# fpthink/PDGN

Measured on AMD Instinct MI355X. Metric: generator+D step points/sec (B=35, 256->2048 pts), higher is better.
Workload: dtype f32; 1 GPU; PDGNet_v2 G+D iteration (models/PDGNet_v2.py:171-256), chair-shaped synthetic batch, per-GPU batch 35, 256->2048 pts, random-init weights; global_batch=35, parallelism=dp1, losses_finite=True, hipgraph=False, issue=list

## Files before the change

include/pdgn_hip.h:

```cpp
#ifndef PDGN_HIP_H
#define PDGN_HIP_H

#include <stdint.h>

#ifdef __cplusplus
extern "C" {
#endif

#define PDGN_ERR_INVALID (-1)
#define PDGN_KNN_MAX_NSAMPLE 200

typedef void *pdgn_stream_t;

#define PDGN_ABI_VERSION 38
int pdgn_abi_version(void);

int pdgn_knnquery(int b, int n, int m, int nsample, const float *xyz, const float *new_xyz,
                  int32_t *idx, float *dist2, pdgn_stream_t stream);

int pdgn_grouping_forward(int b, int c, int n, int m, int nsample, const float *points,
                          const int32_t *idx, float *out, pdgn_stream_t stream);

int pdgn_grouping_backward(int b, int c, int n, int m, int nsample, const float *grad_out,
                           const int32_t *idx, float *grad_points, pdgn_stream_t stream);
// ... 89 lines not shown
int pdgn_dense_bn_maxpool_input_grad(int b, int n, int c, int k, int act, const float *x, const float *dout,
                                     const int32_t *yarg, const float *stats, const float *h, int ldh,
                                     const float *W, int ldw, float *scratch, float *dh, pdgn_stream_t stream);

int pdgn_group_colsum(long long groups, long long group_rows, int c, const float *x, long long ldx, float *out,
                      pdgn_stream_t stream);

int pdgn_softmax_slots_permute(long long m, int k, int c, const float *h, float *w, pdgn_stream_t stream);
int pdgn_bn_softmax_slots_permute(long long m, int k, int c, int act, const float *x, const float *stats,
                                  float *w, pdgn_stream_t stream);
int pdgn_bn_softmax_slots_permute_mul(long long m, int k, int c, int act, const float *x, const float *stats,
                                      int act_u, const float *u, const float *stats_u, float *w, float *y,
                                      unsigned *max_out, const float *gamma_u, const float *beta_u, float bound_scale,
                                      unsigned *cmax_out, pdgn_stream_t stream);
long long pdgn_bilateral_scratch_floats(long long m, int k, int c);
int pdgn_bilateral_weighting_backward(long long m, int k, int c, int act, int training, const float *x,
                                      const float *stats_x, const float *u, const float *stats_u, const float *w,
                                      const float *dy, float *scratch, float *bsums_x, float *bsums_u, float *dx,
                                      float *du, pdgn_stream_t stream);
int pdgn_softmax_slots_permute_backward(long long m, int k, int c, const float *w, const float *dw,
                                        float *dh, pdgn_stream_t stream);

int pdgn_skinny_nt(int R, int N, int K, const float *A, int lda, const float *B, int ldb, const float *bias, float *C, int ldc,
                   pdgn_stream_t stream);
int pdgn_skinny_nn(int R, int N, int K, const float *A, int lda, const float *B, int ldb, float *C, int ldc, pdgn_stream_t stream);
int pdgn_skinny_nt_act(int R, int N, int K, const float *A, int lda, const float *B, int ldb, const float *bias, float *C, int ldc,
                       int act, pdgn_stream_t stream);
int pdgn_skinny_nn_masked(int R, int N, int K, const float *A, int lda, const float *P, int ldp, int act, const float *B,
                          int ldb, float *C, int ldc, pdgn_stream_t stream);
int pdgn_skinny_tn(int R, int N, int K, const float *A, int lda, const float *B, int ldb, float *C, int ldc, pdgn_stream_t stream);
int pdgn_split_bf16x3(int rows, int cols, const float *src, int ld_src, unsigned short *planes, int ld_planes,
                      long long plane_stride, unsigned short *planes_t, int ld_planes_t, long long plane_stride_t,
                      pdgn_stream_t stream);
int pdgn_gemm_nt_ps(long long m, int n, int k, const float *A, int lda, const unsigned short *Wplanes, int ldw, long long wplane,
                    int parts, const float *bias, const float *addend, int ldadd, float *C, int ldc, float *stat_part,
                    const float *row_bias, int ld_rb, int rows_per_group, int act, const float *gate, int ldgate,
                    pdgn_stream_t stream);
long long pdgn_gemm_tail_workspace_floats(long long m, int n, int k, int with_stats);
long long pdgn_gemm_tn_big_workspace_floats(long long m, int n, int k);
int pdgn_gemm_set_tail_workspace(float *ws, long long floats);
int pdgn_gemm_nt_ps_launch_info(long long m, int n, int k, int parts, const void **sym, int *grid);
int pdgn_gemm_aux_symbols(const void **reduce, const void **scan);
int pdgn_gemm_set_mode(int mode);
int pdgn_gemm_set_scale_slots(void *slots, long long bytes);
int pdgn_absmax_rows_cols(long long rows, int cols, const float *src, int ld, unsigned *rowmax, unsigned *colmax,
                          pdgn_stream_t stream);
int pdgn_gemm_set_operand_scales(const unsigned *max_a, const unsigned *max_w);
int pdgn_gemm_two_part(long long m, int n, int k, long long scan_bytes);
int pdgn_gemm_two_part_planes(long long m, int n, int k, long long scan_bytes);
long long pdgn_gemm_nt_ps_stat_rows(long long m, int n, int k, int parts, int plain);
int pdgn_gemm_nt_ps_stat_block_rows(long long m, int n, int k, int parts, int plain);
int pdgn_gemm_nt_ps_row_panel(long long m, int n, int k, int parts, int plain);
long long pdgn_gemm_nt_ps_workspace_floats(long long m, int n, int k, int parts, int with_stats);
int pdgn_split_f16x2(int rows, int cols, const float *src, int ld_src, unsigned short *planes, int ld_planes,
                     long long plane_stride, unsigned short *planes_t, int ld_planes_t, long long plane_stride_t,
                     pdgn_stream_t stream);
int pdgn_gemm_set_config(int cfg);
int pdgn_gemm_set_shape(int shape);
int pdgn_gemm_nt(long long m, int n, int k, const float *A, int lda, const float *W, int ldw,
                 const float *bias, const float *addend, int ldadd, float *C, int ldc, float *stat_part,
                 pdgn_stream_t stream);
long long pdgn_thin_stat_rows(long long m);
int pdgn_thin_stat_block_rows(void);
int pdgn_thin_nt(long long m, int n, int k, const float *X, int ldx, const float *W, int wrs, int wcs,
                 const float *bias, float *Y, int ldy, float *stat_part, pdgn_stream_t stream);
int pdgn_thin_nt_ex(long long m, int n, int k, const float *X, int ldx, const float *W, int wrs, int wcs,
                    const float *bias, float *Y, int ldy, float *stat_part, const float *gate, int ldgate, pdgn_stream_t stream);
int pdgn_thin_tn(long long m, int ta, int wb, const float *A, int lda, const float *B, int ldb, float *O, int osi,
                 int osj, float *sum_a, float *sum_b, pdgn_stream_t stream);
int pdgn_gemm_nn(long long m, int n, int k, const float *A, int lda, const float *Wt, int ldw,
                 const float *bias, const float *addend, int ldadd, float *C, int ldc, float *stat_part,
                 pdgn_stream_t stream);
int pdgn_gemm_tn_big(long long m, int n, int k, const float *dY, int ldy, const float *X, int ldx, float *dW, int dw_is_zero,
                     pdgn_stream_t stream);
int pdgn_gemm_nt_ex(long long m, int n, int k, const float *A, int lda, const float *W, int ldw, const float *bias,
                    const float *addend, int ldadd, float *C, int ldc, float *stat_part, const float *row_bias, int ld_rb,
                    int rows_per_group, int act, const float *gate, int ldgate, int transposed_w, pdgn_stream_t stream);
long long pdgn_gemm_nt_stat_rows(long long m, int n, int k);
int pdgn_gemm_nt_stat_block_rows(long long m, int n, int k);
int pdgn_gemm_nt_config(long long m, int n, int k, int with_stats);

int pdgn_gemm_tn(long long m, int n, int k, const float *dY, const float *X, float *dW,
                 pdgn_stream_t stream);

int pdgn_local_stats(int b, int n, int m, int k, const float *xyz, const int32_t *idx, float *mu,
                     float *cov, pdgn_stream_t stream);
int pdgn_local_stats_backward(int b, int n, int m, int k, const float *xyz, const int32_t *idx,
                              const float *dmu, const float *dcov, float *dxyz, pdgn_stream_t stream);

int pdgn_chamfer_gram(int b, int m, int n, int d, const float *x, const float *y, float *minx,
                      int32_t *argx, float *miny, int32_t *argy, pdgn_stream_t stream);
int pdgn_chamfer_gram_grad(int b, int m, int n, int d, const float *x, const float *y,
                           const float *gminx, const int32_t *argx, const float *gminy,
                           const int32_t *argy, float *gx, float *gy, pdgn_stream_t stream);
int pdgn_chamfer_gram_grad_uniform(int b, int m, int n, int d, const float *x, const float *y, const float *g,
                                   float scale, const int32_t *argx, const int32_t *argy, float *gx, float *gy,
                                   pdgn_stream_t stream);
int pdgn_scaled_sum(long long n, const float *x, float scale, float *out, pdgn_stream_t stream);
int pdgn_mse_const(long long n, const float *x, float target, float scale, float *out, pdgn_stream_t stream);
int pdgn_mse_const_count(long long n, const float *x, float target, float scale, float boundary, float *out, int32_t *count,
                         pdgn_stream_t stream);
int pdgn_mse_const_backward(long long n, const float *x, float target, float scale, const float *g, float *dx,
                            pdgn_stream_t stream);

int pdgn_emd_cost_indexed(int npairs, int n, int m, const float *xyz1, const int32_t *ia,
                          const float *xyz2, const int32_t *ib, float *temp, float *out,
                          pdgn_stream_t stream);
int pdgn_chamfer_gram_indexed(int npairs, int m, int n, int d, const float *x, const int32_t *ia,
                              const float *y, const int32_t *ib, float *minx, int32_t *argx,
                              float *miny, int32_t *argy, pdgn_stream_t stream);

int pdgn_deconv_assemble(int F, int Fo, int k, int T, int fc, const float *Wi, const float *W2, const float *Wf,
                         float *WcatC, float *WcatV, float *Wb, pdgn_stream_t stream);
int pdgn_deconv_assemble_backward(int F, int Fo, int k, int T, int fc, const float *gWcatC, const float *gWcatV,
                                  const float *gWb, float *dWi, float *dW2, float *dWf, pdgn_stream_t stream);

int pdgn_sample_bias(int b, int ldy, int nspec, const int *T, const int *C, const int *off, const int *offc,
                     const float *const *bias, const float *Yc, float *bb, pdgn_stream_t stream);
int pdgn_sample_bias_backward(int b, int ldy, int nspec, const int *T, const int *C, const int *off, const int *offc,
                              const float *g, float *dYc, float *const *dbias, pdgn_stream_t stream);

int pdgn_small_mlp_forward(int r, int k, int n, int act, int bn_mode, float eps, float momentum, const float *x,
                           const float *W, const float *bias, const float *gamma, const float *beta,
                           float *running_mean, float *running_var, float *y, float *pre, float *stat,
                           pdgn_stream_t stream);
int pdgn_small_mlp_backward(int r, int k, int n, int act, int bn_mode, const float *x, const float *dy, const float *pre,
                            const float *stat, const float *gamma, const float *beta, float *dpre, float *dgamma,
                            float *dbeta, float *dbias, float *dW, pdgn_stream_t stream);

int pdgn_ballquery(int b, int n, int m, float radius, int nsample, const float *new_xyz, const float *xyz,
                   int32_t *idx, pdgn_stream_t stream);
int pdgn_furthestsampling(int b, int n, int m, const float *xyz, float *temp, int32_t *idx, pdgn_stream_t stream);
int pdgn_gathering_forward(int b, int c, int n, int m, const float *points, const int32_t *idx, float *out,
                           pdgn_stream_t stream);
int pdgn_gathering_backward(int b, int c, int n, int m, const float *grad_out, const int32_t *idx,
                            float *grad_points, pdgn_stream_t stream);
int pdgn_grouping_int_forward(int b, int c, int n, int m, int nsample, const long long *points, const int32_t *idx,
                              long long *out, pdgn_stream_t stream);
int pdgn_featuredistribute(int b, int n, int m, const float *max_xyz, const float *xyz, int32_t *distribute_idx,
                           pdgn_stream_t stream);
int pdgn_labelstat_idx(int b, int n, int m, int nsample, int nclass, const int32_t *label_stat, const int32_t *idx,
                       int32_t *new_label_stat, pdgn_stream_t stream);
int pdgn_labelstat_ballrange(int b, int n, int m, float radius, int nclass, const float *new_xyz, const float *xyz,
                             const int32_t *label_stat, int32_t *new_label_stat, pdgn_stream_t stream);
int pdgn_labelstat_and_ballquery(int b, int n, int m, float radius, int nsample, int nclass, const float *new_xyz,
                                 const float *xyz, const int32_t *label_stat, int32_t *idx, int32_t *new_label_stat,
                                 pdgn_stream_t stream);

long long pdgn_point_max_scratch(int b, int n, int c);
int pdgn_point_max(int b, int n, int c, const float *x, float *scratch_val, int32_t *scratch_arg, float *out, int32_t *arg,
                   pdgn_stream_t stream);
int pdgn_point_max_backward(int b, int n, int c, const float *grad_out, const int32_t *arg, float *grad_x,
                            pdgn_stream_t stream);

int pdgn_spin(unsigned int microseconds, pdgn_stream_t stream);

int pdgn_replay_marker(int id, pdgn_stream_t stream);
int pdgn_replay_build(void *hip_graph, void **plan_out);
int pdgn_replay_info(void *plan, int *counts8);
int pdgn_replay_chains(void *plan, int *labels, int *nodes_per_chain);
int pdgn_replay_set_stream(void *plan, int chain, pdgn_stream_t stream);
int pdgn_replay_launch(void *plan);
int pdgn_replay_launch_range(void *plan, int lo, int hi);
int pdgn_replay_position(void *plan, int chain, int nth);
int pdgn_replay_points(void *plan, int *ids, int *pos, int *chain, int max_out);
int pdgn_replay_joined(void *plan);
// ... 137 lines not shown
```

pdgn_amd/csrc/gemm_shared.h:

```cpp
#pragma once
#include <type_traits>

#include "common.h"

typedef float f32x4 __attribute__((ext_vector_type(4)));
typedef unsigned u32x4 __attribute__((ext_vector_type(4)));
typedef __attribute__((address_space(3))) void lds_void_t;

#define NT_BK 32
#define NT_GROUP_M 8
#define NT_OOB 0x40000000u

typedef int i32x4 __attribute__((ext_vector_type(4)));

__device__ __forceinline__ i32x4 nt_srd(const void *base, unsigned bytes) {
    const unsigned long long b = (unsigned long long)base;
    i32x4 r;
    r.x = __builtin_amdgcn_readfirstlane((int)(unsigned)b);
    r.y = __builtin_amdgcn_readfirstlane((int)((unsigned)(b >> 32) & 0xffffu));
    r.z = __builtin_amdgcn_readfirstlane((int)bytes);
    r.w = 0x00020000;
    return r;
}

__device__ __forceinline__ void nt_dma16(i32x4 srd, unsigned lds_base, unsigned voff, unsigned soff) {
    asm volatile("s_mov_b32 m0, %0\n\ts_nop 0\n\tbuffer_load_dwordx4 %1, %2, %3 offen lds"
                 :
                 : "s"(lds_base), "v"(voff), "s"(srd), "s"(soff)
                 : "memory", "m0");
}

struct NtArgs {
    long long M;
    int N, K, lda, ldw, ldc, ldadd;
    const float *A, *W, *bias, *addend;
    float *C, *stat_part;
    int tiles_m, tiles_n, tile_begin, tile_end, kchunks;
    long long sk_per_wg;
    int sk_split;
    float *sk_ws;
    int sk_seg;
    int dbg;
    const float *row_bias;
    int ld_rb, rows_per_group;
    unsigned rpg_magic;
    int rb_bytes;
    int act;
    const float *gate;
    int ldgate;
    const unsigned short *Wp;
    long long wplane;
    const unsigned *max_a, *max_w;
};

__device__ __forceinline__ int x2_exponent(unsigned maxbits) {
    const int e = 14 - ((int)(maxbits >> 23) - 127);
    return e > 126 ? 126 : (e < -126 ? -126 : e);
}
__device__ __forceinline__ int x2_scale_field(unsigned maxbits) {
    const int f = 268 - (int)(maxbits >> 23);
    return f < 1 ? 1 : (f > 253 ? 253 : f);
}
__device__ __forceinline__ float x2_scale(unsigned maxbits) { return __int_as_float(x2_scale_field(maxbits) << 23); }
__device__ __forceinline__ float x2_unscale(unsigned maxbits) { return __int_as_float((254 - x2_scale_field(maxbits)) << 23); }

struct NtDev {
    int cus;
};
static inline int nt_cus() {
    static int cached = 0;
    if (!cached) {
        int dev = 0, cus = 0;
        if (hipGetDevice(&dev) != hipSuccess ||
            hipDeviceGetAttribute(&cus, hipDeviceAttributeMultiprocessorCount, dev) != hipSuccess || cus < 1)
            return 256;
        cached = cus;
    }
    return cached;
}

struct NtSwitches {
    int mode, cfg, splitk, shape16, shape16_default;
};
NtSwitches &nt_switches();

struct NtEpi {
    const float *row_bias = nullptr;
    int ld_rb = 0, rows_per_group = 1, act = 0;
    const float *gate = nullptr;
    int ldgate = 0;
    bool any() const { return row_bias || act || gate; }
};


int fp32_gemm_nt(long long m, int n, int k, const float *A, int lda, const float *W, int ldw, const float *bias,
                 const float *addend, int ldadd, float *C, int ldc, float *stat_part, pdgn_stream_t stream);
int fp32_gemm_nn(long long m, int n, int k, const float *A, int lda, const float *Wt, int ldw, const float *bias,
                 const float *addend, int ldadd, float *C, int ldc, float *stat_part, pdgn_stream_t stream);
int fp32_gemm_nt_ex(long long m, int n, int k, const float *A, int lda, const float *W, int ldw, const float *bias,
                    const float *addend, int ldadd, float *C, int ldc, float *stat_part, const float *row_bias, int ld_rb,
                    int rows_per_group, int act, const float *gate, int ldgate, int transposed_w, pdgn_stream_t stream);
int fp32_gemm_tn_big(long long m, int n, int k, const float *dY, int ldy, const float *X, int ldx, float *dW,
                     pdgn_stream_t stream);
long long fp32_gemm_nt_stat_rows(long long m, int n, int k);
int fp32_gemm_nt_stat_block_rows(long long m, int n, int k);
int fp32_gemm_nt_config(long long m, int n, int k, int with_stats);
```

pdgn_amd/csrc/gemm_x3.hip:

```cpp
#include <atomic>
#include <type_traits>

#include "gemm_shared.h"

#ifndef X3_FENCE
#define X3_FENCE 2
#endif
#ifndef X3_DEFAULT_MASK
#define X3_DEFAULT_MASK 0x000
#endif
#ifndef X3_FENCE16
#define X3_FENCE16 2
#endif
#ifndef X3_ABLATE
#define X3_ABLATE 0
#endif

typedef float f32x16 __attribute__((ext_vector_type(16)));
typedef float f32x2 __attribute__((ext_vector_type(2)));
typedef __bf16 bf16x8 __attribute__((ext_vector_type(8)));
typedef __bf16 bf16x2 __attribute__((ext_vector_type(2)));

struct X3Parts {
    u32x4 h, m, l;
};

__device__ __forceinline__ unsigned x3_cvt_pk(float a, float b) {
    const f32x2 v = {a, b};
    return __builtin_bit_cast(unsigned, __builtin_convertvector(v, bf16x2));
}

__device__ __forceinline__ void x3_split_pair(float a, float b, X3Parts &P, int e) {
    const unsigned h = x3_cvt_pk(a, b);
    const float ra = a - __uint_as_float(h << 16), rb = b - __uint_as_float(h & 0xffff0000u);
    const unsigned m = x3_cvt_pk(ra, rb);
    const float sa = ra - __uint_as_float(m << 16), sb = rb - __uint_as_float(m & 0xffff0000u);
    P.h[e] = h;
    P.m[e] = m;
    P.l[e] = x3_cvt_pk(sa, sb);
}

__device__ __forceinline__ f32x16 x3_mfma(const u32x4 a, const u32x4 b, const f32x16 c) {
    return __builtin_amdgcn_mfma_f32_32x32x16_bf16(__builtin_bit_cast(bf16x8, a), __builtin_bit_cast(bf16x8, b), c, 0, 0, 0);
}

typedef _Float16 f16x8 __attribute__((ext_vector_type(8)));
typedef _Float16 f16x2 __attribute__((ext_vector_type(2)));
__device__ __forceinline__ unsigned x2_cvt_pk(float a, float b) {
    const f32x2 v = {a, b};
    return __builtin_bit_cast(unsigned, __builtin_convertvector(v, f16x2));
}
__device__ __forceinline__ f32x16 x2_mfma(const u32x4 a, const u32x4 b, const f32x16 c) {
    return __builtin_amdgcn_mfma_f32_32x32x16_f16(__builtin_bit_cast(f16x8, a), __builtin_bit_cast(f16x8, b), c, 0, 0, 0);
}
#ifndef X2_PRODUCTS
#define X2_PRODUCTS 3
#endif

typedef float f32x4a __attribute__((ext_vector_type(4)));
__device__ __forceinline__ f32x4a x3_mfma16(const u32x4 a, const u32x4 b, const f32x4a c) {
    return __builtin_amdgcn_mfma_f32_16x16x32_bf16(__builtin_bit_cast(bf16x8, a), __builtin_bit_cast(bf16x8, b), c, 0, 0, 0);
}

template <int MS>
__device__ __forceinline__ unsigned x3_sw(unsigned r) {
    const unsigned x = (r >> 2) & 3u;
    return MS == 32 ? x : ((0x78u >> (2u * x)) & 3u);
}

template <int CTRL, int ROW_MASK>
__device__ __forceinline__ float x3_dpp_add(float v) {
    return v + __int_as_float(__builtin_amdgcn_update_dpp(0, __float_as_int(v), CTRL, ROW_MASK, 0xf, true));
}

__device__ __forceinline__ float x3_half_wave_sum(float v) {
    v = x3_dpp_add<0x111, 0xf>(v);
    v = x3_dpp_add<0x112, 0xf>(v);
    v = x3_dpp_add<0x114, 0xf>(v);
    v = x3_dpp_add<0x118, 0xf>(v);
    return x3_dpp_add<0x142, 0xa>(v);
}

__device__ __forceinline__ float x3_row_sum(float v) {
    v = x3_dpp_add<0x111, 0xf>(v);
    v = x3_dpp_add<0x112, 0xf>(v);
    v = x3_dpp_add<0x114, 0xf>(v);
    return x3_dpp_add<0x118, 0xf>(v);
}

template <int TM, int TN, int WM, int WN, int OCC, bool ATOMIC, bool WT, bool AT, bool EPI = false, bool PW = false, int MS = 32, int NP = 3>
__global__ __launch_bounds__(64 * WM * WN, OCC) void gemm_x3_kernel(const NtArgs p) {
    static_assert(!PW || (!WT && !AT), "pre-split second operand: row-major (N x K) planes only");
    static_assert(MS == 32 || MS == 16, "matrix instruction: 32x32x16 or 16x16x32");
    static_assert(NP == 3 || (NP == 2 && MS == 32), "parts: three bf16, or two fp16 on the 32x32x16 instruction");
    constexpr int NW = WM * WN, NTH = 64 * NW, BM = 32 * TM * WM, BN = 32 * TN * WN;
    constexpr int PART_A = BM * 64, PART_W = BN * 64, STAGE = NP * (PART_A + PART_W);
    constexpr int UNT = NP == 2 ? (BM + BN) * 4 : 0;
    constexpr bool STG = OCC == 1 && !ATOMIC && !(X3_ABLATE & 128) && 2 * STAGE + NW * 4096 + UNT <= 160 * 1024;
    __shared__ __attribute__((aligned(1024))) unsigned char smem[2 * STAGE + (STG ? NW * 4096 : 0) + UNT];
    float *const untab = reinterpret_cast<float *>(smem + 2 * STAGE + (STG ? NW * 4096 : 0));

    const int tid = threadIdx.x, lane = tid & 63;
    const int wave = __builtin_amdgcn_readfirstlane(tid >> 6);
    const int wm = wave / WN, wn = wave % WN;
    const int li = MS == 32 ? lane & 31 : lane & 15, lg = MS == 32 ? lane >> 5 : lane >> 4;

    const int G = gridDim.x, pid = blockIdx.x;
    const int gq = G >> 3, gr = G & 7, xcd = pid & 7;
    const int v = xcd * gq + min(xcd, gr) + (pid >> 3);

    const int KC = p.kchunks;
    auto decode = [&](int tile, int &tm, int &tn) {
        const int per_group = NT_GROUP_M * p.tiles_n;
        const int grp = tile / per_group, r = tile - grp * per_group;
        const int first = grp * NT_GROUP_M;
        const int gsz = min(NT_GROUP_M, p.tiles_m - first);
        tn = r / gsz;
        tm = first + (r - tn * gsz);
    };
    struct Cur {
        int tile, kb, kc, ke;
        int j;
        long long f, f1;
        bool valid;
    };
    auto next_item = [&](Cur &c) {
        if (p.sk_split && (ATOMIC || p.sk_ws)) {
// ... 1479 lines not shown
```

pdgn_amd/fused.py:

```python
import os
import weakref

import torch
from ._fn import Function

from . import _lib
from ._lib import check, ptr, require, stream_of

F32 = torch.float32
ACT = {"none": 0, "relu": 1, "leaky_relu": 2}


def _scratch_floats(L, rows, C):
    n = L.pdgn_bn_scratch_floats(rows, C)
    if n < 0:
        raise _lib.PdgnHipError("pdgn_bn_scratch_floats: argument outside the supported range")
    return n


_ZERO_COLSUM = {}


def mark_zero_colsum(dx):
    _ZERO_COLSUM[dx.data_ptr()] = weakref.ref(dx)
# ... 157 lines not shown
def _pre_bias_grad(ctx_has, C, device):
    return _zeros((C,), device) if ctx_has else None


class BNActCL(Function):

    @staticmethod
    def forward(ctx, x, gamma, beta, running_mean, running_var, training, momentum, eps, act, mul, pre_bias=None,
                partials=None, interleave_n=0):
        rows, C = x.shape
        x = x.contiguous()
        L = _lib.lib()
        g, b = gamma.detach().contiguous(), beta.detach().contiguous()
        stats = _bn_stats(L, x, rows, C, g, b, pre_bias, running_mean, running_var, training, momentum, eps, partials)
        ctx.has_pre_bias = pre_bias is not None
        mul_c = mul.contiguous() if mul is not None else None
        y = torch.empty((rows * 2, C // 2), dtype=F32, device=x.device) if interleave_n else torch.empty_like(x)
        check(L.pdgn_bn_act_forward(rows, C, act, ptr(x), ptr(stats), ptr(mul_c), ptr(y), int(interleave_n), stream_of(x)), "pdgn_bn_act_forward")
        ctx.save_for_backward(x, stats, mul_c)
        ctx.cfg = (rows, C, act, bool(training), mul is not None and mul.requires_grad, int(interleave_n))
        return y

    @staticmethod
    def backward(ctx, dy):
        x, stats, mul = ctx.saved_tensors
        rows, C, act, training, need_dmul, inter = ctx.cfg
        dy = dy.contiguous()
        L = _lib.lib()
        scratch = torch.empty(_scratch_floats(L, rows, C), dtype=F32, device=x.device)
        bs = torch.empty(2 * C, dtype=F32, device=x.device)
        dx = torch.empty_like(x)
        dmul = torch.empty_like(x) if need_dmul else None
        check(L.pdgn_bn_act_backward(rows, C, act, int(training), ptr(x), ptr(dy), ptr(mul),
                                     ptr(stats), ptr(scratch), ptr(bs), ptr(dx), ptr(dmul), inter, stream_of(x)), "pdgn_bn_act_backward")
        if training:
            mark_zero_colsum(dx)
        return (dx, bs[C:], bs[:C], None, None, None, None, None, None, dmul, _pre_bias_grad(ctx.has_pre_bias, C, x.device),
                None, None)


_PENDING_COUNTS = {}
_HOLD_COUNTS = [False]


def hold_bn_counters(on):
    old, _HOLD_COUNTS[0] = _HOLD_COUNTS[0], bool(on)
    return old


def flush_bn_counters():
    if _HOLD_COUNTS[0]:
        return
    if _PENDING_COUNTS:
        tensors = list(_PENDING_COUNTS.keys())
        torch._foreach_add_(tensors, [int(v) for v in _PENDING_COUNTS.values()])
        _PENDING_COUNTS.clear()


def bn_act(x2d, bn, training, act="leaky_relu", mul=None, pre_bias=None, partials=None, interleave_n=0):
    if training and bn.track_running_stats:
        _PENDING_COUNTS[bn.num_batches_tracked] = _PENDING_COUNTS.get(bn.num_batches_tracked, 0) + 1
    x2d, pre_bias = _fold_pre_bias(x2d, pre_bias, training)
    if x2d.shape[1] % 4:
        if pre_bias is not None:
            x2d = x2d + pre_bias
        y = torch.nn.functional.batch_norm(x2d, bn.running_mean, bn.running_var, bn.weight, bn.bias, training,
                                           bn.momentum, bn.eps)
        y = {"none": lambda t: t, "relu": torch.relu, "leaky_relu": torch.nn.functional.leaky_relu}[act](y)
        y = y * mul if mul is not None else y
        return interleave_rows(y, interleave_n) if interleave_n else y
    if interleave_n and (mul is not None or not x2d.is_cuda):
        return interleave_rows(bn_act(x2d, bn, training, act, mul, pre_bias, partials), interleave_n)
    return BNActCL.apply(x2d, bn.weight, bn.bias, bn.running_mean, bn.running_var, training, bn.momentum, bn.eps,
                         ACT[act], mul, pre_bias, partials, interleave_n)


def interleave_rows(y2d, n):
    rows, c2 = y2d.shape
    return y2d.view(rows // n, n, c2 // 2, 2).permute(0, 3, 1, 2).reshape(rows * 2, c2 // 2)


_OWN_MIN_ROWS = 1024
_TN_BIG = os.environ.get("PDGN_TN_BIG", "1") == "1"


def _tn_big_max():
    return (1 << 22) if _lib.matrix_core_mode() else (1 << 20)


def _pad_cols(t, mult=4):
    c = t.shape[1]
    if c % mult == 0 and t.stride(1) == 1 and t.stride(0) % 4 == 0 and t.data_ptr() % 16 == 0:
        return t
    if c % mult == 0:
        return t.contiguous()
    return torch.nn.functional.pad(t, (0, mult - c % mult)).contiguous()


GEMM_LOG = None


_PLANES = os.environ.get("PDGN_PLANES", "1") == "1"


class Planes:
    __slots__ = ("p", "t", "shape", "parts_p", "parts_t")

    def __init__(self, p, t, shape, parts_p=3, parts_t=3):
        self.p, self.t, self.shape, self.parts_p, self.parts_t = p, t, shape, parts_p, parts_t


def two_part(m, n, k, scan_bytes):
    return _lib.gemm_mode() == "x2" and bool(_lib.lib().pdgn_gemm_two_part(m, n, k, scan_bytes))


def two_part_planes(m, n, k, scan_bytes):
    return _lib.gemm_mode() == "x2" and bool(_lib.lib().pdgn_gemm_two_part_planes(m, n, k, scan_bytes))


def _slots(t):
    if _lib.gemm_mode() == "x2":
        _lib.ensure_scale_slots(t.device)


def split_planes(w, want_t, rows=None, dy_maxima_free=False, x_maxima_free=False):
    _slots(w)
    mode = _lib.gemm_mode()
    if (not (_PLANES and w.is_cuda and w.dim() == 2 and mode != "fp32") or w.shape[0] % 4 or w.shape[1] % 4 or w.stride(1) != 1
            or w.stride(0) % 4 or w.data_ptr() % 16):
        return None
    n, k = w.shape
    ldp, ldt = (k + 7) // 8 * 8, (n + 7) // 8 * 8
    parts_p = 2 if rows and two_part_planes(rows, n, k, 0 if x_maxima_free else rows * k * 4) else 3
    parts_t = 2 if rows and want_t and two_part_planes(rows, k, n, 0 if dy_maxima_free else rows * n * 4) else 3

    def planes(parts, rows_, ld):
        buf = torch.empty(parts * rows_ * ld + 2 * rows_ + 8, dtype=torch.int16, device=w.device)
        return buf[:parts * rows_ * ld].view(parts, rows_, ld)
    P = planes(parts_p, n, ldp)
    PT = planes(parts_t, k, ldt) if want_t else None
    L = _lib.lib()
    st = stream_of(w)
    if parts_p == parts_t or not want_t:
        fn = L.pdgn_split_bf16x3 if parts_p == 3 else L.pdgn_split_f16x2
        check(fn(n, k, ptr(w), w.stride(0), ptr(P), ldp, n * ldp, ptr(PT), ldt, k * ldt if want_t else 0, st), "pdgn_split")
    else:
        for parts, args in ((parts_p, (ptr(P), ldp, n * ldp, None, 0, 0)),
                            (parts_t, (None, 0, 0, ptr(PT), ldt, k * ldt))):
            fn = L.pdgn_split_bf16x3 if parts == 3 else L.pdgn_split_f16x2
            check(fn(n, k, ptr(w), w.stride(0), *args, st), "pdgn_split")
    return Planes(P, PT, (n, k), parts_p, parts_t)


def _maxima_ok(t):
    return (_lib.gemm_mode() == "x2" and t.is_cuda and t.dim() == 2 and t.stride(1) == 1 and t.dtype == F32 and t.shape[1] % 4 == 0
            and t.stride(0) % 4 == 0 and t.data_ptr() % 16 == 0)


def operand_maxima(t, rows=True, cols=False):
    if not _maxima_ok(t) or not (rows or cols):
        return (None, None) if (rows and cols) else None
    rm = torch.empty((t.shape[0],), dtype=torch.int32, device=t.device) if rows else None
    cm = torch.empty((t.shape[1],), dtype=torch.int32, device=t.device) if cols else None
    check(_lib.lib().pdgn_absmax_rows_cols(t.shape[0], t.shape[1], ptr(t), t.stride(0), ptr(rm), ptr(cm), stream_of(t)), "pdgn_absmax_rows_cols")
    return (rm, cm) if (rows and cols) else (rm if rows else cm)

# ... 9 lines not shown

def _tail_workspace(L, m, n, k, with_stats, device, parts=None):
    if parts is not None:
        need = L.pdgn_gemm_nt_ps_workspace_floats(m, n, k, parts, 1 if with_stats else 0)
    else:
        need = L.pdgn_gemm_tail_workspace_floats(m, n, k, 1 if with_stats else 0)
    if need <= 0:
        return None
    ws = torch.empty(need, dtype=F32, device=device)
    check(L.pdgn_gemm_set_tail_workspace(ptr(ws), need), "pdgn_gemm_set_tail_workspace")
    return ws


def _rp_takes(m, n, k, parts, plain):
    return parts == 2 and plain and _lib.lib().pdgn_gemm_nt_ps_row_panel(m, n, k, 2, 1) == 1


def planes_fit(P, m, n, k, with_stats=False, plain=False):
    return (P.shape[0] == 3 or not with_stats or _rp_takes(m, n, k, P.shape[0], plain) or (_lib.lib().pdgn_gemm_nt_config(m, n, k, 1) & 15) == 0)


def gemm_nt_planes(a, P, n, k, bias=None, addend=None, want_stats=False, max_a=None):
    _slots(a)
    m = a.shape[0]
    if GEMM_LOG is not None:
        GEMM_LOG.append(("nt", m, n, k))
    ap = _pad_cols(a)
    L = _lib.lib()
    out = torch.empty((m, n), dtype=F32, device=a.device)
    part = None
    if want_stats:
        part = torch.empty((L.pdgn_gemm_nt_ps_stat_rows(m, n, k, P.shape[0], 1 if (bias is None and addend is None) else 0),
                            3 * n), dtype=F32, device=a.device)
    b = bias.detach().contiguous() if bias is not None else None
    if addend is not None:
        addend = _pad_cols(addend)
    ws = _tail_workspace(L, m, n, k, want_stats, a.device, parts=P.shape[0])
    _hand_maxima(L, max_a)
    check(L.pdgn_gemm_nt_ps(m, n, k, ptr(ap), ap.stride(0), ptr(P), P.shape[2], P.shape[1] * P.shape[2], P.shape[0],
                            ptr(b), ptr(addend), addend.stride(0) if addend is not None else 0, ptr(out), n, ptr(part), None, 0, 1, 0,
                            None, 0, stream_of(a)), "pdgn_gemm_nt_ps")
    return (out, part) if want_stats else out


def gemm_nt(a, w, bias=None, addend=None, want_stats=False, w_transposed=False, max_a=None):
    _slots(a)
    m, k = a.shape
    n = w.shape[1] if w_transposed else w.shape[0]
    if GEMM_LOG is not None:
        GEMM_LOG.append(("nn" if w_transposed else "nt", m, n, k))
    ap = _pad_cols(a)
    kp = ap.shape[1]
    np_ = (n + 3) // 4 * 4
    if w_transposed:
        wp = _pad_cols(w)
        if kp != k:
            wp = torch.nn.functional.pad(wp, (0, 0, 0, kp - k))
    else:
        wp = _pad_cols(w)
    if np_ != n and not w_transposed:
        wp = torch.nn.functional.pad(wp, (0, 0, 0, np_ - n))
    if np_ != n:
        bias = torch.nn.functional.pad(bias, (0, np_ - n)) if bias is not None else None
        addend = torch.nn.functional.pad(addend, (0, np_ - n)) if addend is not None else None
    if addend is not None:
        addend = _pad_cols(addend)
    L = _lib.lib()
    out = torch.empty((m, np_), dtype=F32, device=a.device)
    part = None
    if want_stats:
        part = torch.empty((L.pdgn_gemm_nt_stat_rows(m, np_, kp), 3 * np_), dtype=F32, device=a.device)
    b = bias.detach().contiguous() if bias is not None else None
    fn = L.pdgn_gemm_nn if w_transposed else L.pdgn_gemm_nt
    ws = _tail_workspace(L, m, np_, kp, want_stats, a.device)
    _hand_maxima(L, max_a)
    check(fn(m, np_, kp, ptr(ap), ap.stride(0), ptr(wp), wp.stride(0), ptr(b), ptr(addend),
             addend.stride(0) if addend is not None else 0, ptr(out), np_, ptr(part), stream_of(a)),
          "pdgn_gemm_nn" if w_transposed else "pdgn_gemm_nt")
    if np_ != n:
        out = out[:, :n].contiguous()
    return (out, part) if want_stats else out


def gemm_tn(dy, x, max_dy=None, max_x=None):
    _slots(dy)
    m, n = dy.shape
    k = x.shape[1]
    if GEMM_LOG is not None:
        GEMM_LOG.append(("tn", m, n, k))
    dyp, xp = _pad_cols(dy), _pad_cols(x)
    nk = dyp.shape[1] * xp.shape[1]
    if _TN_BIG and dyp.shape[1] >= 64 and xp.shape[1] >= 64 and (65536 if (m < 150000 or not _lib.matrix_core_mode()) else 16384) <= nk <= _tn_big_max():
        L = _lib.lib()
        need = L.pdgn_gemm_tn_big_workspace_floats(m, dyp.shape[1], xp.shape[1])
        if need > 0:
            ws = torch.empty(need, dtype=F32, device=dy.device)
            check(L.pdgn_gemm_set_tail_workspace(ptr(ws), need), "pdgn_gemm_set_tail_workspace")
            dwp = torch.empty((dyp.shape[1], xp.shape[1]), dtype=F32, device=dy.device)
        else:
            dwp = _zeros((dyp.shape[1], xp.shape[1]), dy.device)
        _hand_maxima(L, max_dy, max_x)
        check(_lib.lib().pdgn_gemm_tn_big(m, dyp.shape[1], xp.shape[1], ptr(dyp), dyp.stride(0), ptr(xp),
                                          xp.stride(0), ptr(dwp), 0 if need > 0 else 1, stream_of(dy)), "pdgn_gemm_tn_big")
        return dwp if (dyp.shape[1] == n and xp.shape[1] == k) else dwp[:n, :k]
    if dyp.stride(0) != dyp.shape[1]:
        dyp = dyp.contiguous()
    if xp.stride(0) != xp.shape[1]:
        xp = xp.contiguous()
    dwp = _zeros((dyp.shape[1], xp.shape[1]), dy.device)
    check(_lib.lib().pdgn_gemm_tn(m, dyp.shape[1], xp.shape[1], ptr(dyp), ptr(xp), ptr(dwp), stream_of(dy)), "pdgn_gemm_tn")
    return dwp if (dyp.shape[1] == n and xp.shape[1] == k) else dwp[:n, :k]


def _thin_ok(x, n, k):
    return (k <= 4 and n % 4 == 0 and n <= 1024) or (n <= 4 and k % 4 == 0 and k <= 1024)


def thin_nt(x, w, wrs, wcs, n, bias=None, want_stats=False):
    m, k = x.shape
    if GEMM_LOG is not None:
        GEMM_LOG.append(("thin", m, n, k))
    x = x if (x.stride(1) == 1 and (k <= 4 or (x.stride(0) % 4 == 0 and x.data_ptr() % 16 == 0))) else x.contiguous()
    L = _lib.lib()
    out = torch.empty((m, n), dtype=F32, device=x.device)
    part = None
    if want_stats and k <= 4:
        part = torch.empty((L.pdgn_thin_stat_rows(m), 3 * n), dtype=F32, device=x.device)
    b = bias.detach().contiguous() if bias is not None else None
    check(L.pdgn_thin_nt(m, n, k, ptr(x), x.stride(0), ptr(w), wrs, wcs, ptr(b), ptr(out), n, ptr(part), stream_of(x)), "pdgn_thin_nt")
    return (out, part) if want_stats else out


def thin_tn(dy, x, want_db):
    m, n = dy.shape
    k = x.shape[1]
    if GEMM_LOG is not None:
        GEMM_LOG.append(("thin_tn", m, n, k))
    dw = _zeros((n, k), dy.device)
    db = _zeros((n,), dy.device) if want_db else None
    L = _lib.lib()
    if k <= 4:
        check(L.pdgn_thin_tn(m, k, n, ptr(x), x.stride(0), ptr(dy), dy.stride(0), ptr(dw), 1, k, ptr(None), ptr(db), stream_of(dy)), "pdgn_thin_tn")
    else:
        check(L.pdgn_thin_tn(m, n, k, ptr(dy), dy.stride(0), ptr(x), x.stride(0), ptr(dw), k, 1, ptr(db), ptr(None), stream_of(dy)), "pdgn_thin_tn")
    return dw, db


def _planes_taken(x, weight, planes, want_stats, plain):
    return (planes is not None and x.is_cuda and x.shape[0] >= _PLANES_MIN_ROWS and planes.shape == tuple(weight.shape)
            and x.shape[1] == weight.shape[1] and x.shape[1] % 4 == 0
            and planes_fit(planes.p, x.shape[0], weight.shape[0], weight.shape[1], want_stats, plain))


class LinearCL(Function):

    @staticmethod
    def forward(ctx, x, weight, bias, addend, want_stats=False, planes=None, x_max=None, x_cmax=None):
        ctx.save_for_backward(x, weight)
        ctx.set_materialize_grads(False)
        ctx.has_bias = bias is not None
        ctx.has_addend = addend is not None
        ctx.planes_t = None
        ctx.max_x = None
        ctx.max_x_cols = x_cmax
        if _planes_taken(x, weight, planes, want_stats, bias is None and addend is None):
            n, k = weight.shape
            ctx.thin = False
            ctx.planes_t = planes.t
            xm = None
            if planes.parts_p == 2 and not _rp_takes(x.shape[0], n, k, 2, bias is None and addend is None):
                xm = x_max if x_max is not None else operand_maxima(x)
            ctx.max_x = xm
            if want_stats:
                y, part = gemm_nt_planes(x, planes.p, n, k, bias, addend, want_stats=True, max_a=xm)
                ctx.mark_non_differentiable(part)
                return y, part
            return gemm_nt_planes(x, planes.p, n, k, bias, addend, max_a=xm)
        ctx.thin = bool(x.is_cuda and x.shape[0] >= _OWN_MIN_ROWS and addend is None and weight.is_contiguous()
                        and _thin_ok(x, weight.shape[0], weight.shape[1]))
        if ctx.thin:
            n, k = weight.shape
            if want_stats and k <= 4:
                y, part = thin_nt(x, weight, k, 1, n, bias, want_stats=True)
                ctx.mark_non_differentiable(part)
                return y, part
            y = thin_nt(x, weight, k, 1, n, bias)
# ... 646 lines not shown
```

Measured before the change: 3.147 million points/s.

## Add split-K bf16x3 MFMA weight-gradient GEMM for small TN shapes

Adds a new TN GEMM kernel for weight gradients outside the existing big-TN route. It splits each fp32 input into three bf16 parts and accumulates six MFMA cross products, which aims for near-fp32 accuracy on the matrix cores. It also splits the long M reduction across workgroups, writing to a workspace that a separate reduce kernel sums. The goal is to replace the old scalar pdgn_gemm_tn path with better CU occupancy and matrix-core throughput, at the cost of an extra reduction launch, workspace allocation and conversion work.

After: 3.145 million points/s. Within noise of the previous version (-0.1%).

```diff
diff --git a/include/pdgn_hip.h b/include/pdgn_hip.h
--- a/include/pdgn_hip.h
+++ b/include/pdgn_hip.h
@@ -195,6 +195,10 @@
 
 int pdgn_gemm_tn(long long m, int n, int k, const float *dY, const float *X, float *dW,
                  pdgn_stream_t stream);
+int pdgn_gemm_tn_sp(long long m, int n, int k, const float *dY, int ldy, const float *X, int ldx, float *dW, int lddw,
+                    float *workspace, long long workspace_floats, pdgn_stream_t stream);
+long long pdgn_gemm_tn_sp_workspace_floats(long long m, int n, int k);
+int pdgn_gemm_tn_sp_plan(long long m, int n, int k, int *tile_n, int *tile_k, int *splits, long long *rows_per_split);
 
 int pdgn_local_stats(int b, int n, int m, int k, const float *xyz, const int32_t *idx, float *mu,
                      float *cov, pdgn_stream_t stream);
diff --git a/pdgn_amd/csrc/gemm_shared.h b/pdgn_amd/csrc/gemm_shared.h
--- a/pdgn_amd/csrc/gemm_shared.h
+++ b/pdgn_amd/csrc/gemm_shared.h
@@ -64,6 +64,34 @@
 __device__ __forceinline__ float x2_scale(unsigned maxbits) { return __int_as_float(x2_scale_field(maxbits) << 23); }
 __device__ __forceinline__ float x2_unscale(unsigned maxbits) { return __int_as_float((254 - x2_scale_field(maxbits)) << 23); }
 
+typedef float f32x16 __attribute__((ext_vector_type(16)));
+typedef float f32x2 __attribute__((ext_vector_type(2)));
+typedef __bf16 bf16x8 __attribute__((ext_vector_type(8)));
+typedef __bf16 bf16x2 __attribute__((ext_vector_type(2)));
+
+struct X3Parts {
+    u32x4 h, m, l;
+};
+
+__device__ __forceinline__ unsigned x3_cvt_pk(float a, float b) {
+    const f32x2 v = {a, b};
+    return __builtin_bit_cast(unsigned, __builtin_convertvector(v, bf16x2));
+}
+
+__device__ __forceinline__ void x3_split_pair(float a, float b, X3Parts &P, int e) {
+    const unsigned h = x3_cvt_pk(a, b);
+    const float ra = a - __uint_as_float(h << 16), rb = b - __uint_as_float(h & 0xffff0000u);
+    const unsigned m = x3_cvt_pk(ra, rb);
+    const float sa = ra - __uint_as_float(m << 16), sb = rb - __uint_as_float(m & 0xffff0000u);
+    P.h[e] = h;
+    P.m[e] = m;
+    P.l[e] = x3_cvt_pk(sa, sb);
+}
+
+__device__ __forceinline__ f32x16 x3_mfma(const u32x4 a, const u32x4 b, const f32x16 c) {
+    return __builtin_amdgcn_mfma_f32_32x32x16_bf16(__builtin_bit_cast(bf16x8, a), __builtin_bit_cast(bf16x8, b), c, 0, 0, 0);
+}
+
 struct NtDev {
     int cus;
 };
diff --git a/pdgn_amd/csrc/gemm_tn_sp.hip b/pdgn_amd/csrc/gemm_tn_sp.hip
--- /dev/null
+++ b/pdgn_amd/csrc/gemm_tn_sp.hip
@@ -0,0 +1,324 @@
+#include "gemm_shared.h"
+
+typedef short sp_s16x4 __attribute__((ext_vector_type(4)));
+typedef __attribute__((address_space(3))) sp_s16x4 sp_lds_s16x4;
+
+#define SP_THREADS 256
+#define SP_MIN_ROWS 64
+#define SP_MAX_BLOCKS 16
+
+struct SpArgs {
+    long long M, rows;
+    int N, K, ldy, ldx, lddw;
+    int tiles_n, tiles_k, splits;
+    int ws_ld;
+    long long ws_split;
+    const float *dY, *X;
+    float *dW, *ws;
+};
+
+__host__ __device__ constexpr int sp_pitch(int t) { return ((2 * t) % 256 == 64 || (2 * t) % 256 == 192) ? 2 * t : 2 * t + 64; }
+
+__device__ __forceinline__ void sp_split4(const float4 v, uint2 &h, uint2 &m, uint2 &l) {
+    X3Parts P;
+    x3_split_pair(v.x, v.y, P, 0);
+    x3_split_pair(v.z, v.w, P, 1);
+    h = make_uint2(P.h[0], P.h[1]);
+    m = make_uint2(P.m[0], P.m[1]);
+    l = make_uint2(P.l[0], P.l[1]);
+}
+
+template <int PITCH>
+__device__ __forceinline__ u32x4 sp_frag(const unsigned char *p) {
+    const sp_s16x4 lo = __builtin_amdgcn_ds_read_tr16_b64_v4i16((sp_lds_s16x4 *)p);
+    const sp_s16x4 hi = __builtin_amdgcn_ds_read_tr16_b64_v4i16((sp_lds_s16x4 *)(p + 4 * PITCH));
+    const uint2 a = __builtin_bit_cast(uint2, lo), b = __builtin_bit_cast(uint2, hi);
+    u32x4 r = {a.x, a.y, b.x, b.y};
+    return r;
+}
+
+template <int TN, int TK, int CH>
+__global__ __launch_bounds__(SP_THREADS, (TN / 32) * ((TK < 32 ? 32 : TK) / 32) >= SP_MAX_BLOCKS ? 3 : 4) void gemm_tn_sp_kernel(const SpArgs a) {
+    constexpr int TKB = TK < 32 ? 32 : TK;
+    constexpr int BN = TN / 32, BK = TKB / 32;
+    constexpr int WGN = (BN >= 4 && BK >= 4) ? 2 : (BN >= 4 ? 4 : (BK >= 8 ? 1 : BN));
+    constexpr int WGK = (4 / WGN) < BK ? (4 / WGN) : BK;
+    constexpr int WBN = BN / WGN, WBK = BK / WGK;
+    constexpr int PY = sp_pitch(TN), PX = sp_pitch(TKB);
+    constexpr int QY = TN / 4, QX = TK / 4;
+    constexpr int YSTEP = SP_THREADS / QY, XSTEP = SP_THREADS / QX;
+    constexpr int NY = (CH + YSTEP - 1) / YSTEP, NX = (CH + XSTEP - 1) / XSTEP;
+    static_assert(BN * BK <= SP_MAX_BLOCKS && WBN * WGN == BN && WBK * WGK == BK, "tile");
+    __shared__ __attribute__((aligned(16))) unsigned char Ys[3 * CH * PY];
+    __shared__ __attribute__((aligned(16))) unsigned char Xs[3 * CH * PX];
+
+    const int total = gridDim.x, pid = blockIdx.x;
+    const int q8 = total >> 3, r8 = total & 7, xcd = pid & 7, slot = pid >> 3;
+    const int v = xcd * q8 + min(xcd, r8) + slot;
+    const int tiles = a.tiles_n * a.tiles_k;
+    const int tile = v % tiles, split = v / tiles;
+    const int n0 = (tile % a.tiles_n) * TN, k0 = (tile / a.tiles_n) * TK;
+    const long long m_begin = (long long)split * a.rows;
+    const long long m_end = min(a.M, m_begin + a.rows);
+
+    const int tid = threadIdx.x, lane = tid & 63, wave = tid >> 6;
+    const int wn = wave / WGK, wk = wave % WGK;
+    const bool multiplies = wave < WGN * WGK;
+
+    const int yr = tid / QY, yq = tid % QY, xr = tid / QX, xq = tid % QX;
+    const bool ycol = n0 + 4 * yq < a.N, xcol = k0 + 4 * xq < a.K;
+    const float *pY = a.dY + (m_begin + yr) * a.ldy + n0 + 4 * yq;
+    const float *pX = a.X + (m_begin + xr) * a.ldx + k0 + 4 * xq;
+    float4 ry[NY], rx[NX];
+    auto prefetch = [&](long long m0, bool tail) {
+#pragma unroll
+        for (int i = 0; i < NY; ++i) {
+            const int row = yr + i * YSTEP;
+            const bool ok = row < CH && ycol && (!tail || m0 + row < m_end);
+            ry[i] = ok ? *reinterpret_cast<const float4 *>(pY + (long long)(i * YSTEP) * a.ldy) : make_float4(0.f, 0.f, 0.f, 0.f);
+        }
+#pragma unroll
+        for (int i = 0; i < NX; ++i) {
+            const int row = xr + i * XSTEP;
+            const bool ok = row < CH && xcol && (!tail || m0 + row < m_end);
+            rx[i] = ok ? *reinterpret_cast<const float4 *>(pX + (long long)(i * XSTEP) * a.ldx) : make_float4(0.f, 0.f, 0.f, 0.f);
+        }
+    };
+
+    f32x16 acc[WBN][WBK];
+#pragma unroll
+    for (int i = 0; i < WBN; ++i)
+#pragma unroll
+        for (int j = 0; j < WBK; ++j)
+#pragma unroll
+            for (int r = 0; r < 16; ++r) acc[i][j][r] = 0.f;
+
+    const int fg = lane >> 5, fc = (lane >> 4) & 1, fq = (lane >> 2) & 3, fp = lane & 3;
+    const unsigned char *fY = Ys + (8 * fg + fq) * PY + (32 * wn * WBN + 16 * fc + 4 * fp) * 2;
+    const unsigned char *fX = Xs + (8 * fg + fq) * PX + (32 * wk * WBK + 16 * fc + 4 * fp) * 2;
+
+    const long long span = m_end - m_begin;
+    const int nfull = (int)(span / CH), nchunk = (int)((span + CH - 1) / CH);
+    prefetch(m_begin, nfull == 0);
+    for (int c = 0; c < nchunk; ++c) {
+        __syncthreads();
+#pragma unroll
+        for (int i = 0; i < NY; ++i) {
+            const int row = yr + i * YSTEP;
+            if (row < CH) {
+                uint2 h, m, l;
+                sp_split4(ry[i], h, m, l);
+                unsigned char *d = Ys + row * PY + yq * 8;
+                *reinterpret_cast<uint2 *>(d) = h;
+                *reinterpret_cast<uint2 *>(d + CH * PY) = m;
+                *reinterpret_cast<uint2 *>(d + 2 * CH * PY) = l;
+            }
+        }
+#pragma unroll
+        for (int i = 0; i < NX; ++i) {
+            const int row = xr + i * XSTEP;
+            if (row < CH) {
+                uint2 h, m, l;
+                sp_split4(rx[i], h, m, l);
+                unsigned char *d = Xs + row * PX + xq * 8;
+                *reinterpret_cast<uint2 *>(d) = h;
+                *reinterpret_cast<uint2 *>(d + CH * PX) = m;
+                *reinterpret_cast<uint2 *>(d + 2 * CH * PX) = l;
+            }
+        }
+        __syncthreads();
+        pY += (long long)CH * a.ldy;
+        pX += (long long)CH * a.ldx;
+        if (c + 1 < nchunk) prefetch(m_begin + (long long)(c + 1) * CH, c + 1 >= nfull);
+        if (multiplies) {
+#pragma unroll
+            for (int s = 0; s < CH / 16; ++s) {
+                u32x4 yf[WBN][3], xf[WBK][3];
+#pragma unroll
+                for (int p = 0; p < 3; ++p) {
+#pragma unroll
+                    for (int i = 0; i < WBN; ++i) yf[i][p] = sp_frag<PY>(fY + (p * CH + 16 * s) * PY + 64 * i);
+#pragma unroll
+                    for (int j = 0; j < WBK; ++j) xf[j][p] = sp_frag<PX>(fX + (p * CH + 16 * s) * PX + 64 * j);
+                }
+                constexpr int PA[6] = {2, 1, 0, 1, 0, 0}, PB[6] = {0, 1, 2, 0, 1, 0};
+#pragma unroll
+                for (int t = 0; t < 6; ++t)
+#pragma unroll
+                    for (int i = 0; i < WBN; ++i)
+#pragma unroll
+                        for (int j = 0; j < WBK; ++j) acc[i][j] = x3_mfma(xf[j][PA[t]], yf[i][PB[t]], acc[i][j]);
+            }
+        }
+    }
+    if (!multiplies) return;
+    float *out = a.ws ? a.ws + (long long)split * a.ws_split : a.dW;
+    const int ldo = a.ws ? a.ws_ld : a.lddw;
+#pragma unroll
+    for (int i = 0; i < WBN; ++i) {
+        const int n = n0 + 32 * (wn * WBN + i) + (lane & 31);
+        if (!a.ws && n >= a.N) continue;
+#pragma unroll
+        for (int j = 0; j < WBK; ++j)
+#pragma unroll
+            for (int e = 0; e < 4; ++e) {
+                const int kl = 32 * (wk * WBK + j) + 8 * e + 4 * fg;
+                if (kl >= TK || (!a.ws && k0 + kl >= a.K)) continue;
+                const float4 o = make_float4(acc[i][j][4 * e], acc[i][j][4 * e + 1], acc[i][j][4 * e + 2], acc[i][j][4 * e + 3]);
+                *reinterpret_cast<float4 *>(out + (long long)n * ldo + k0 + kl) = o;
+            }
+    }
+}
+
+__global__ __launch_bounds__(256) void gemm_tn_sp_reduce_kernel(const float *__restrict__ ws, int S, long long ws_split, int ws_ld,
+                                                                int N, int K, float *__restrict__ dW, int lddw, int G) {
+    __shared__ float4 red[256];
+    const int E = 256 / G, k4 = K / 4;
+    const int e = blockIdx.x * E + (int)threadIdx.x % E, g = (int)threadIdx.x / E;
+    const bool in = e < N * k4;
+    const int n = in ? e / k4 : 0, kq = in ? e % k4 : 0;
+    const float *p = ws + (long long)n * ws_ld + 4 * kq;
+    float4 s = make_float4(0.f, 0.f, 0.f, 0.f);
+    if (in && g < S) {
+        s = *reinterpret_cast<const float4 *>(p + (long long)g * ws_split);
+#pragma unroll 4
+        for (int sl = g + G; sl < S; sl += G) {
+            const float4 b = *reinterpret_cast<const float4 *>(p + (long long)sl * ws_split);
+            s.x += b.x; s.y += b.y; s.z += b.z; s.w += b.w;
+        }
+    }
+    if (G > 1) {
+        red[threadIdx.x] = s;
+        __syncthreads();
+        if (g == 0)
+            for (int gg = 1; gg < G; ++gg) {
+                const float4 b = red[gg * E + (int)threadIdx.x];
+                s.x += b.x; s.y += b.y; s.z += b.z; s.w += b.w;
+            }
+    }
+    if (in && g == 0) *reinterpret_cast<float4 *>(dW + (long long)n * lddw + 4 * kq) = s;
+}
+
+struct SpPlan {
+    int tn, tk, tiles_n, tiles_k, splits;
+    long long rows;
+};
+
+static inline long long sp_round(long long v, long long to) { return (v + to - 1) / to * to; }
+
+static SpPlan sp_plan(long long m, int n, int k, int cus) {
+    static const int cand[12][2] = {{128, 128}, {256, 64}, {64, 256}, {128, 64}, {64, 128}, {256, 32},
+                                    {64, 64},   {128, 32}, {256, 16}, {64, 32},  {128, 16}, {64, 16}};
+    long long best_area = -1;
+    for (const auto &c : cand) {
+        const long long area = sp_round(n, c[0]) * sp_round(k, c[1]);
+        if (best_area < 0 || area < best_area) best_area = area;
+    }
+    const long long max_splits = m / SP_MIN_ROWS > 1 ? m / SP_MIN_ROWS : 1;
+    int pick = -1;
+    long long pick_wgs = -1;
+    for (int i = 0; i < 12; ++i) {
+        const long long area = sp_round(n, cand[i][0]) * sp_round(k, cand[i][1]);
+        if (area * 8 > best_area * 9) continue;
+        const long long wgs = (long long)cdiv(n, cand[i][0]) * cdiv(k, cand[i][1]) * max_splits;
+        if (wgs >= cus) { pick = i; break; }
+        if (wgs > pick_wgs) { pick = i; pick_wgs = wgs; }
+    }
+    SpPlan p;
+    p.tn = cand[pick][0];
+    p.tk = cand[pick][1];
+    p.tiles_n = cdiv(n, p.tn);
+    p.tiles_k = cdiv(k, p.tk);
+    const long long tiles = (long long)p.tiles_n * p.tiles_k;
+    long long splits = 2 * cus / tiles;
+    splits = splits > max_splits ? max_splits : splits;
+    splits = splits < 1 ? 1 : splits;
+    long long rows = sp_round((m + splits - 1) / splits, 32);
+    if (rows < SP_MIN_ROWS) rows = SP_MIN_ROWS;
+    while (rows > SP_MIN_ROWS && (m + rows - 33) / (rows - 32) <= max_splits && tiles * ((m + rows - 33) / (rows - 32)) <= 2LL * cus)
+        rows -= 32;
+    p.rows = rows;
+    p.splits = (int)((m + rows - 1) / rows);
+    return p;
+}
+
+template <int TN, int TK>
+static int sp_launch(const SpArgs &a, hipStream_t s) {
+    constexpr int CH = (TN / 32) * ((TK < 32 ? 32 : TK) / 32) >= SP_MAX_BLOCKS / 2 ? 16 : 32;
+    const long long total = (long long)a.tiles_n * a.tiles_k * a.splits;
+    if (total > 0x7fffffffLL) return PDGN_ERR_INVALID;
+    hipLaunchKernelGGL((gemm_tn_sp_kernel<TN, TK, CH>), dim3((unsigned)total), dim3(SP_THREADS), 0, s, a);
+    return pdgn_launch_status();
+}
+
+static bool sp_valid(long long m, int n, int k) {
+    return m >= 1 && n >= 4 && k >= 4 && n % 4 == 0 && k % 4 == 0 && (long long)n * k <= (1LL << 28);
+}
+
+extern "C" int pdgn_gemm_tn_sp_plan(long long m, int n, int k, int *tile_n, int *tile_k, int *splits, long long *rows_per_split) {
+    if (!sp_valid(m, n, k)) return PDGN_ERR_INVALID;
+    const SpPlan p = sp_plan(m, n, k, nt_cus());
+    if (tile_n) *tile_n = p.tn;
+    if (tile_k) *tile_k = p.tk;
+    if (splits) *splits = p.splits;
+    if (rows_per_split) *rows_per_split = p.rows;
+    return 0;
+}
+
+extern "C" long long pdgn_gemm_tn_sp_workspace_floats(long long m, int n, int k) {
+    if (!sp_valid(m, n, k)) return -1;
+    const SpPlan p = sp_plan(m, n, k, nt_cus());
+    return p.splits > 1 ? (long long)p.splits * p.tiles_n * p.tn * p.tiles_k * p.tk : 0;
+}
+
+extern "C" int pdgn_gemm_tn_sp(long long m, int n, int k, const float *dY, int ldy, const float *X, int ldx, float *dW, int lddw,
+                               float *workspace, long long workspace_floats, pdgn_stream_t stream) {
+    if (!sp_valid(m, n, k) || !dY || !X || !dW || ldy < n || ldx < k || lddw < k || ldy % 4 || ldx % 4 || lddw % 4 ||
+        ((uintptr_t)dY | (uintptr_t)X | (uintptr_t)dW | (uintptr_t)workspace) % 16)
+        return PDGN_ERR_INVALID;
+    const SpPlan p = sp_plan(m, n, k, nt_cus());
+    SpArgs a;
+    a.M = m;
+    a.rows = p.rows;
+    a.N = n;
+    a.K = k;
+    a.ldy = ldy;
+    a.ldx = ldx;
+    a.lddw = lddw;
+    a.tiles_n = p.tiles_n;
+    a.tiles_k = p.tiles_k;
+    a.splits = p.splits;
+    a.ws_ld = p.tiles_k * p.tk;
+    a.ws_split = (long long)p.tiles_n * p.tn * a.ws_ld;
+    a.dY = dY;
+    a.X = X;
+    a.dW = dW;
+    a.ws = nullptr;
+    if (p.splits > 1) {
+        if (!workspace || workspace_floats < a.ws_split * p.splits) return PDGN_ERR_INVALID;
+        a.ws = workspace;
+    }
+    hipStream_t s = (hipStream_t)stream;
+    int rc = PDGN_ERR_INVALID;
+    switch (p.tn * 1000 + p.tk) {
+        case 128128: rc = sp_launch<128, 128>(a, s); break;
+        case 256064: rc = sp_launch<256, 64>(a, s); break;
+        case 64256: rc = sp_launch<64, 256>(a, s); break;
+        case 128064: rc = sp_launch<128, 64>(a, s); break;
+        case 64128: rc = sp_launch<64, 128>(a, s); break;
+        case 256032: rc = sp_launch<256, 32>(a, s); break;
+        case 64064: rc = sp_launch<64, 64>(a, s); break;
+        case 128032: rc = sp_launch<128, 32>(a, s); break;
+        case 256016: rc = sp_launch<256, 16>(a, s); break;
+        case 64032: rc = sp_launch<64, 32>(a, s); break;
+        case 128016: rc = sp_launch<128, 16>(a, s); break;
+        case 64016: rc = sp_launch<64, 16>(a, s); break;
+    }
+    if (rc != 0 || p.splits == 1) return rc;
+    const long long elems = (long long)n * (k / 4);
+    int G = 1;
+    while (G < 32 && 2 * G <= p.splits && (elems * G + 255) / 256 < 2LL * nt_cus()) G *= 2;
+    hipLaunchKernelGGL(gemm_tn_sp_reduce_kernel, dim3((unsigned)((elems * G + 255) / 256)), dim3(256), 0, s, a.ws, p.splits, a.ws_split,
+                       a.ws_ld, n, k, dW, lddw, G);
+    return pdgn_launch_status();
+}
diff --git a/pdgn_amd/csrc/gemm_x3.hip b/pdgn_amd/csrc/gemm_x3.hip
--- a/pdgn_amd/csrc/gemm_x3.hip
+++ b/pdgn_amd/csrc/gemm_x3.hip
@@ -16,33 +16,6 @@
 #define X3_ABLATE 0
 #endif
 
-typedef float f32x16 __attribute__((ext_vector_type(16)));
-typedef float f32x2 __attribute__((ext_vector_type(2)));
-typedef __bf16 bf16x8 __attribute__((ext_vector_type(8)));
-typedef __bf16 bf16x2 __attribute__((ext_vector_type(2)));
-
-struct X3Parts {
-    u32x4 h, m, l;
-};
-
-__device__ __forceinline__ unsigned x3_cvt_pk(float a, float b) {
-    const f32x2 v = {a, b};
-    return __builtin_bit_cast(unsigned, __builtin_convertvector(v, bf16x2));
-}
-
-__device__ __forceinline__ void x3_split_pair(float a, float b, X3Parts &P, int e) {
-    const unsigned h = x3_cvt_pk(a, b);
-    const float ra = a - __uint_as_float(h << 16), rb = b - __uint_as_float(h & 0xffff0000u);
-    const unsigned m = x3_cvt_pk(ra, rb);
-    const float sa = ra - __uint_as_float(m << 16), sb = rb - __uint_as_float(m & 0xffff0000u);
-    P.h[e] = h;
-    P.m[e] = m;
-    P.l[e] = x3_cvt_pk(sa, sb);
-}
-
-__device__ __forceinline__ f32x16 x3_mfma(const u32x4 a, const u32x4 b, const f32x16 c) {
-    return __builtin_amdgcn_mfma_f32_32x32x16_bf16(__builtin_bit_cast(bf16x8, a), __builtin_bit_cast(bf16x8, b), c, 0, 0, 0);
-}
 
 typedef _Float16 f16x8 __attribute__((ext_vector_type(8)));
 typedef _Float16 f16x2 __attribute__((ext_vector_type(2)));
diff --git a/pdgn_amd/fused.py b/pdgn_amd/fused.py
--- a/pdgn_amd/fused.py
+++ b/pdgn_amd/fused.py
@@ -263,6 +263,7 @@
 
 _OWN_MIN_ROWS = 1024
 _TN_BIG = os.environ.get("PDGN_TN_BIG", "1") == "1"
+_TN_SP = os.environ.get("PDGN_TN_SP", "1") == "1"
 
 
 def _tn_big_max():
@@ -438,6 +439,13 @@
     return (out, part) if want_stats else out
 
 
+def tn_route(m, n, k):
+    nk = n * k
+    if _TN_BIG and n >= 64 and k >= 64 and (65536 if (m < 150000 or not _lib.matrix_core_mode()) else 16384) <= nk <= _tn_big_max():
+        return "big"
+    return "sp" if _TN_SP and _lib.matrix_core_mode() else "tn"
+
+
 def gemm_tn(dy, x, max_dy=None, max_x=None):
     _slots(dy)
     m, n = dy.shape
@@ -445,8 +453,8 @@
     if GEMM_LOG is not None:
         GEMM_LOG.append(("tn", m, n, k))
     dyp, xp = _pad_cols(dy), _pad_cols(x)
-    nk = dyp.shape[1] * xp.shape[1]
-    if _TN_BIG and dyp.shape[1] >= 64 and xp.shape[1] >= 64 and (65536 if (m < 150000 or not _lib.matrix_core_mode()) else 16384) <= nk <= _tn_big_max():
+    route = tn_route(m, dyp.shape[1], xp.shape[1])
+    if route == "big":
         L = _lib.lib()
         need = L.pdgn_gemm_tn_big_workspace_floats(m, dyp.shape[1], xp.shape[1])
         if need > 0:
@@ -458,6 +466,14 @@
         _hand_maxima(L, max_dy, max_x)
         check(_lib.lib().pdgn_gemm_tn_big(m, dyp.shape[1], xp.shape[1], ptr(dyp), dyp.stride(0), ptr(xp),
                                           xp.stride(0), ptr(dwp), 0 if need > 0 else 1, stream_of(dy)), "pdgn_gemm_tn_big")
+        return dwp if (dyp.shape[1] == n and xp.shape[1] == k) else dwp[:n, :k]
+    if route == "sp":
+        L = _lib.lib()
+        need = L.pdgn_gemm_tn_sp_workspace_floats(m, dyp.shape[1], xp.shape[1])
+        ws = torch.empty(need, dtype=F32, device=dy.device) if need > 0 else None
+        dwp = torch.empty((dyp.shape[1], xp.shape[1]), dtype=F32, device=dy.device)
+        check(L.pdgn_gemm_tn_sp(m, dyp.shape[1], xp.shape[1], ptr(dyp), dyp.stride(0), ptr(xp), xp.stride(0), ptr(dwp),
+                                xp.shape[1], ptr(ws), max(need, 0), stream_of(dy)), "pdgn_gemm_tn_sp")
         return dwp if (dyp.shape[1] == n and xp.shape[1] == k) else dwp[:n, :k]
     if dyp.stride(0) != dyp.shape[1]:
         dyp = dyp.contiguous()
```
